# facebook/zstd

Hardware: NVIDIA H100
Metric: compress GB/s (input) at level 1 (higher is better)
Workload: dtype u8

## Files before the change

zstd_b200/csrc/zb_device.cuh:

```cuda
#ifndef ZB_DEVICE_CUH
#define ZB_DEVICE_CUH
#include <cuda_runtime.h>
#include "zb_common.h"

#define ZB_FULL 0xFFFFFFFFu

__device__ __forceinline__ u32 zb_ld32u(const u8* p)
{
    const u32* q = (const u32*)((uintptr_t)p & ~(uintptr_t)3);
    u32 const sh = ((u32)(uintptr_t)p & 3u) * 8u;
    u32 const a = __ldg(q);
    u32 const b = __ldg(sh ? q + 1 : q);
    return __funnelshift_r(a, b, sh);
}
__device__ __forceinline__ u64 zb_ld64u(const u8* p)
{
    const u32* q = (const u32*)((uintptr_t)p & ~(uintptr_t)3);
    u32 const sh = ((u32)(uintptr_t)p & 3u) * 8u;
    u32 const a = __ldg(q);
    u32 const b = __ldg(q + 1);
    u32 const c = __ldg(sh ? q + 2 : q + 1);
    u32 const lo = __funnelshift_r(a, b, sh);
    u32 const hi = __funnelshift_r(b, c, sh);
    return ((u64)hi << 32) | lo;
}

__device__ __forceinline__ u32 zb_ld32w2(const u8* p)
{
    const u32* q = (const u32*)((uintptr_t)p & ~(uintptr_t)3);
    u32 const sh = ((u32)(uintptr_t)p & 3u) * 8u;
    return __funnelshift_r(__ldg(q), __ldg(q + 1), sh);
}
__device__ __forceinline__ u64 zb_ld64w3(const u8* p)
{
    const u32* q = (const u32*)((uintptr_t)p & ~(uintptr_t)3);
    u32 const sh = ((u32)(uintptr_t)p & 3u) * 8u;
    u32 const a = __ldg(q), b = __ldg(q + 1), c = __ldg(q + 2);
    return ((u64)__funnelshift_r(b, c, sh) << 32) | __funnelshift_r(a, b, sh);
}
struct ZbSeg { const u8* lo; const u8* hi; u32 split; };

template <bool DICT> __device__ __forceinline__ const u8* zb_seg_ptr(const ZbSeg& s, u32 rel)
{
    if (DICT) return (rel < s.split ? s.lo : s.hi) + rel;
    return s.hi + rel;
}
template <bool DICT> __device__ __forceinline__ u8 zb_seg_byte(const ZbSeg& s, u32 rel) { return *zb_seg_ptr<DICT>(s, rel); }

template <bool DICT> __device__ __forceinline__ u64 zb_seg_ld64(const ZbSeg& s, u32 rel)
{
    if (DICT && rel < s.split && rel + 12u > s.split) {
        u64 v = 0;
#pragma unroll
        for (u32 i = 0; i < 8u; i++) v |= (u64)zb_seg_byte<true>(s, rel + i) << (8u * i);
        return v;
    }
    return zb_ld64w3(zb_seg_ptr<DICT>(s, rel));
}
template <bool DICT> __device__ __forceinline__ u64 zb_seg_ld64x(const ZbSeg& s, u32 rel)
{
    if (DICT && rel < s.split && rel + 12u > s.split) {
        u64 v = 0;
#pragma unroll
        for (u32 i = 0; i < 8u; i++) v |= (u64)zb_seg_byte<true>(s, rel + i) << (8u * i);
        return v;
    }
    return zb_ld64u(zb_seg_ptr<DICT>(s, rel));
}
template <bool DICT> __device__ __forceinline__ u32 zb_seg_ld32(const ZbSeg& s, u32 rel) { return (u32)zb_seg_ld64<DICT>(s, rel); }
template <bool DICT> __device__ __forceinline__ void zb_seg_pre_cur(const ZbSeg& sg, u32 x, u32* pre, u32* cur)
{
    u32 const s = x >= 4u ? 0u : 4u - x;
    u64 const w = zb_seg_ld64<DICT>(sg, x + s - 4u);
    *pre = (u32)(w << (8u * s));
    *cur = (u32)(w >> (32u - 8u * s));
}

__device__ __forceinline__ u32 zb_hash(u64 v, u32 mls, u32 hBits)
{
    switch (mls) {
    default:
    case 4: return ((u32)v * 2654435761u) >> (32 - hBits);
    case 5: return (u32)(((v << 24) * 889523592379ull) >> (64 - hBits));
    case 6: return (u32)(((v << 16) * 227718039650203ull) >> (64 - hBits));
    case 7: return (u32)(((v << 8) * 58295818150454627ull) >> (64 - hBits));
    case 8: return (u32)((v * 0xCF1BBCDCB7A56463ull) >> (64 - hBits));
    }
}

__device__ __forceinline__ u32 zb_hb32(u32 v) { return 31u - (u32)__clz((int)v); }

__device__ __forceinline__ u64 zbx_rotl(u64 x, int r) { return (x << r) | (x >> (64 - r)); }
#define ZBX_P1 0x9E3779B185EBCA87ull
#define ZBX_P2 0xC2B2AE3D27D4EB4Full
#define ZBX_P3 0x165667B19E3779F9ull
#define ZBX_P4 0x85EBCA77C2B2AE63ull
#define ZBX_P5 0x27D4EB2F165667C5ull
__device__ __forceinline__ u64 zbx_round(u64 acc, u64 in) { return zbx_rotl(acc + in * ZBX_P2, 31) * ZBX_P1; }
__device__ __forceinline__ u64 zbx_merge(u64 h, u64 v) { return (h ^ zbx_round(0, v)) * ZBX_P1 + ZBX_P4; }

#endif
```

zstd_b200/csrc/zb_match.cu:

```cuda
#include "zb_device.cuh"
#include "zb_kernels.h"
#include "zb_merge.cuh"

#ifndef WALK_FAST_BC
#define WALK_FAST_BC 1
#endif

template <bool DICT>
__device__ __forceinline__ u32 zb_count_fwd(const ZbSeg& sg, u32 a, u32 offset, u32 be, u32 lane)
{
    u32 fwd = 0;
    while (true) {
        u32 const pa = a + fwd + 8u * lane;
        u32 m;
        if (pa + 8u <= be) {
            u64 const x = zb_seg_ld64x<DICT>(sg, pa) ^ zb_seg_ld64x<DICT>(sg, pa - offset);
            m = x ? (u32)((__ffsll((long long)x) - 1) >> 3) : 8u;
        } else {
            m = 0;
            while (pa + m < be && zb_seg_byte<DICT>(sg, pa + m) == zb_seg_byte<DICT>(sg, pa + m - offset)) m++;
        }
        u32 const inc = __ballot_sync(ZB_FULL, m != 8u);
        if (inc == 0) { fwd += 256u; continue; }
        int const f = __ffs((int)inc) - 1;
        fwd += 8u * (u32)f + __shfl_sync(ZB_FULL, m, f);
        return fwd;
    }
}

template <bool DICT>
__device__ __forceinline__ u32 zb_back_coop(const ZbSeg& sg, u32 probe, u32 offset, u32 anchor, u32 lane)
{
    u32 back = 0;
    while (true) {
        u32 const k = back + lane + 1u;
        bool const ok = (probe >= anchor + k) && (probe >= offset + k)
                     && (zb_seg_byte<DICT>(sg, probe - k) == zb_seg_byte<DICT>(sg, probe - offset - k));
        u32 const okb = __ballot_sync(ZB_FULL, ok);
        u32 const cnt = (okb == ZB_FULL) ? 32u : (u32)(__ffs((int)~okb) - 1);
        back += cnt;
        if (cnt < 32u) return back;
    }
}

__device__ __forceinline__ u64 zb_pack_raw(u32 off, u32 mlen, u32 msRel) { return (u64)off | ((u64)mlen << 24) | ((u64)msRel << 42); }
#define ZB_RAW_OFF(r)  ((u32)(r) & 0xFFFFFFu)
#define ZB_RAW_MLEN(r) ((u32)((r) >> 24) & 0x3FFFFu)
#define ZB_RAW_MS(r)   ((u32)((r) >> 42))

#define ZB_TAG_MASK ((1u << ZB_TAG_BITS) - 1u)
__device__ __forceinline__ u32 zb_walk_key(u32 x) { return (x | (ZB_BATCH - 1u)) - (x & (ZB_BATCH - 1u)); }
__device__ __forceinline__ u32 zb_walk_entry(u32 h, u32 x) { return ((zb_walk_key(x) + 1u) << ZB_TAG_BITS) | (h & ZB_TAG_MASK); }
__device__ __forceinline__ u32 zb_walk_cand(u32 c, u32 h, u32 x)
{
    u32 const px = zb_walk_key((c >> ZB_TAG_BITS) - 1u);
    return (((c ^ h) & ZB_TAG_MASK) == 0u && px < x) ? x - px : 0u;
}

template <int P>
__device__ __forceinline__ u32 zb_walk_pattern_res(u32 r0, u32 step)
{
    if (step <= 2u) return (1u << P) - 1u;
    u32 m = 3u >> (r0 < 2u ? r0 : 2u);
    u32 nxt = step - r0;
#pragma unroll
    for (int k = 0; k < (P + 2) / 3; k++) {
        m |= 3u << (nxt < 31u ? nxt : 31u);
        nxt += step;
    }
    return m & ((1u << P) - 1u);
}
__device__ __forceinline__ u32 zb_walk_residue(u32 rel0, u32 step)
{
    u32 const q = (u32)__fdividef((float)rel0, (float)step);
    int r = (int)rel0 - (int)(q * step);
    if (r < 0) r += (int)step; else if (r >= (int)step) r -= (int)step;
    return (u32)r;
}

#define ZB_WALK_NWR(P) ((P) == 1 ? 2 : ((P) + 7 + 3) / 4)
template <int MLS, int P, bool INTERIOR>
__device__ __forceinline__ bool zb_walk_batch(u32* __restrict__ table, u32 xa, const u32 (&wrd)[ZB_WALK_NWR(P)], u32 pat,
                                              u32 N, u32 shift, u32 D, u32 total, u32 xLow, u32 xEnd,
                                              const u8* fbase, const u8* dbase, bool output, u16* __restrict__ distRow, u32* __restrict__ farRow)
{
    u32 h[P], bkt[P], dOld[P];
    bool act[P];
    {   u32 const rel0 = xa - shift;
        bool const slow = !INTERIOR && ((xa < xLow) || (D != 0u && rel0 < D && rel0 + P + 7u > D) || (rel0 + P + 7u > total));
        u32 old[P];
#pragma unroll
        for (int i = 0; i < P; i++) {
            u32 const x = xa + (u32)i, rel = x - shift;
            act[i] = INTERIOR ? true : ((x >= xLow) && (rel + 8u <= total) && !(rel < D && rel + 8u > D));
            u64 v;
            if (slow) v = act[i] ? zb_ld64u((rel < D ? dbase : fbase) + rel) : 0ull;
            else {
                constexpr int NWR = ZB_WALK_NWR(P);
                int const wi = i >> 2; u32 const sh = 8u * (u32)(i & 3);
                int const w2 = wi + 2 < NWR ? wi + 2 : NWR - 1;
                u32 const lo = (i & 3) ? __funnelshift_r(wrd[wi], wrd[wi + 1], sh) : wrd[wi];
                u32 const hi = (i & 3) ? __funnelshift_r(wrd[wi + 1], wrd[w2], sh) : wrd[wi + 1];
                v = ((u64)hi << 32) | lo;
            }
            h[i] = zb_hash(v, MLS, 32u);
            bkt[i] = __umulhi(h[i], N);
            old[i] = act[i] ? table[bkt[i]] : 0u;
        }
#pragma unroll
        for (int i = 0; i < P; i++) dOld[i] = zb_walk_cand(old[i], h[i], xa + (u32)i);
    }
    u32 anyOld = 0;
#pragma unroll
    for (int i = 0; i < P; i++) anyOld |= dOld[i];
    bool const anyHit = __syncthreads_or(anyOld != 0u) != 0;
#if WALK_FAST_BC
    u32 const Y1 = zb_walk_key(xa) + 1u;
#pragma unroll
    for (int i = 0; i < P; i++)
        if (act[i] && dOld[i] == 0u && ((pat >> i) & 1u)) atomicMax(&table[bkt[i]], ((Y1 - (u32)i) << ZB_TAG_BITS) | (h[i] & ZB_TAG_MASK));
    __syncthreads();
    u32 d[P];
#pragma unroll
    for (int i = 0; i < P; i++) {
        d[i] = dOld[i];
        if (act[i] && d[i] == 0u) {
            u32 const c = table[bkt[i]];
            int const dd = (int)((c >> ZB_TAG_BITS) - Y1 + (u32)i);
            d[i] = ((((c ^ h[i]) & ZB_TAG_MASK) == 0u) && dd > 0) ? (u32)dd : 0u;
        }
    }
#else
#pragma unroll
    for (int i = 0; i < P; i++)
        if (act[i] && dOld[i] == 0u && ((pat >> i) & 1u)) atomicMax(&table[bkt[i]], zb_walk_entry(h[i], xa + (u32)i));
    __syncthreads();
    u32 d[P];
#pragma unroll
    for (int i = 0; i < P; i++) {
        d[i] = dOld[i];
        if (act[i] && d[i] == 0u) d[i] = zb_walk_cand(table[bkt[i]], h[i], xa + (u32)i);
    }
#endif
    if (output && (INTERIOR || xa < xEnd)) {
        u32 anyFar = 0;
#pragma unroll
        for (int i = 0; i < P; i++) anyFar |= d[i] >= ZB_FAR ? 1u : 0u;
        if (anyFar) {
#pragma unroll
            for (int i = 0; i < P; i++) if (d[i] >= ZB_FAR) { if (INTERIOR || xa + (u32)i < xEnd) farRow[i] = d[i]; d[i] = ZB_FAR; }
        }
        bool vec = false;
        if constexpr (P == 16) { if (INTERIOR || xa + 16u <= xEnd) { uint4* const o4 = reinterpret_cast<uint4*>(distRow);
                                     o4[0] = make_uint4(d[0] | (d[1] << 16), d[2] | (d[3] << 16), d[4] | (d[5] << 16), d[6] | (d[7] << 16));
                                     o4[1] = make_uint4(d[8] | (d[9] << 16), d[10] | (d[11] << 16), d[12] | (d[13] << 16), d[14] | (d[15] << 16)); vec = true; } }
        if constexpr (P == 8) { if (INTERIOR || xa + 8u <= xEnd) { *reinterpret_cast<uint4*>(distRow) = make_uint4(d[0] | (d[1] << 16), d[2] | (d[3] << 16), d[4] | (d[5] << 16), d[6] | (d[7] << 16)); vec = true; } }
        if constexpr (P == 4) { if (INTERIOR || xa + 4u <= xEnd) { *reinterpret_cast<uint2*>(distRow) = make_uint2(d[0] | (d[1] << 16), d[2] | (d[3] << 16)); vec = true; } }
        if constexpr (P == 2) { if (INTERIOR || xa + 2u <= xEnd) { *reinterpret_cast<u32*>(distRow) = d[0] | (d[1] << 16); vec = true; } }
        if (!vec) {
#pragma unroll
            for (int i = 0; i < P; i++) if (xa + (u32)i < xEnd) distRow[i] = (u16)d[i];
        }
    }
    return anyHit;
}

#ifndef WALK_STEADY
#define WALK_STEADY 1
#endif
#ifndef WALK_P_SMALL
#define WALK_P_SMALL 8
#endif
#ifndef WALK_P_MID
#define WALK_P_MID 4
#endif
#ifndef WALK_MINB_SMALL
#define WALK_MINB_SMALL 4
#endif
template <int MLS, int P>
__global__ void __launch_bounds__(ZB_BATCH / P, P == WALK_P_SMALL ? WALK_MINB_SMALL : 1)
zb_walk_kernel(const u8* __restrict__ src, const u8* __restrict__ dictEnd, const ZbChunk* __restrict__ chunks, u32 insStep, u32 N, ZbStrides sd,
               u32 slotFirstBlock, u16* __restrict__ dist, u32* __restrict__ far,
               const u32* __restrict__ imageIn, u32* __restrict__ imageOut)
{
    constexpr u32 THREADS = ZB_BATCH / P;
    extern __shared__ __align__(16) u32 table[];
    u32 const t = threadIdx.x;
    ZbChunk const cd = chunks[blockIdx.x];
    bool const buildImage = imageOut != nullptr;
    u32 const D = cd.dictLen;
    u32 const H = cd.histLen;
    u32 const total = buildImage ? D : H + cd.size;
    bool const fromImage = imageIn != nullptr && D != 0u && !buildImage;
    u32 const shift = (ZB_BATCH - (D % ZB_BATCH)) % ZB_BATCH;
    const u8* const fbase = src + cd.srcOff - H;
    const u8* const dbase = dictEnd - D;

    if (fromImage) for (u32 i = t; i < N; i += THREADS) table[i] = __ldg(imageIn + i);
    else           for (u32 i = t; i < N; i += THREADS) table[i] = 0u;
    __syncthreads();

    u32 const xEnd = total + shift;
    u32 const xLow = (fromImage ? D : 0u) + shift;
    u32 x0 = xLow & ~(ZB_BATCH - 1u);
    u32 const xIntLo = ((D + shift) > xLow ? (D + shift) : xLow);
    u32 const xIntLoB = (xIntLo + ZB_BATCH - 1u) & ~(ZB_BATCH - 1u);
    constexpr u32 NW = (P + 7u + 3u + 3u) / 4u;
    constexpr int NWR = ZB_WALK_NWR(P);
    u32 const xIntHi = xEnd >= (ZB_BATCH + 4u * NW) ? (xEnd + P - 4u * NW) & ~(ZB_BATCH - 1u) : 0u;

    auto fetch = [&](u32 xb, u32 (&a)[NW], u32& sh) {
        u32 const xa = xb + P * t;
#pragma unroll
        for (u32 k = 0; k < NW; k++) a[k] = 0u;
        sh = 0u;
        if (xb >= xIntLoB && xb + ZB_BATCH <= xIntHi) {
            const u8* const ad = fbase + (xa - shift);
            const u32* const p = reinterpret_cast<const u32*>((uintptr_t)ad & ~(uintptr_t)3);
            sh = ((u32)(uintptr_t)ad & 3u) * 8u;
#pragma unroll
            for (u32 k = 0; k < NW; k++) a[k] = __ldg(p + k);
            return;
        }
        if (xa + P <= xLow || xa >= xEnd) return;
        u32 const rel = xa - shift;
        bool const slow = (xa < xLow) || (D != 0u && rel < D && rel + P + 7u > D) || (rel + P + 7u > total);
        if (slow) return;
        const u8* const ad = (rel < D ? dbase : fbase) + rel;
        const u32* const p = reinterpret_cast<const u32*>((uintptr_t)ad & ~(uintptr_t)3);
        u32 const al = (u32)(uintptr_t)ad & 3u;
        sh = al * 8u;
#pragma unroll
        for (u32 k = 0; k < NW; k++) a[k] = (al + P + 7u > 4u * k) ? __ldg(p + k) : 0u;
    };
    u32 rawA[NW], rawB[NW], shA, shB;
    fetch(x0, rawA, shA);
    fetch(x0 + ZB_BATCH, rawB, shB);
    u32 const blockMask = (1u << cd.blockLog) - 1u;
    u32 const stepInc = ZB_BATCH % insStep;
    u32 r0 = (x0 + P * t + insStep * ZB_BATCH - shift) % insStep;
    u32 li = shift;
    auto doBatch = [&](u32 (&raw)[NW], u32& sh) {
        u32 const xa = x0 + P * t;
        u32 cur[NWR];
#pragma unroll
        for (int k = 0; k < NWR; k++) cur[k] = __funnelshift_r(raw[k], (u32)k + 1u < NW ? raw[(u32)k + 1u < NW ? k + 1 : k] : 0u, sh);
        fetch(x0 + 2u * ZB_BATCH, raw, sh);
        if (D != 0u && x0 >= D + shift && li < D + shift) li = D + shift;
        u32 const sWalk = x0 > xLow ? x0 : xLow;
        u32 const step = insStep + ((sWalk - li) >> 7);
        u32 const pat = zb_walk_pattern_res<P>(step == insStep ? r0 : zb_walk_residue(xa - shift, step), step);
        bool const output = !buildImage && x0 >= H + shift;
        u32 const qb0 = x0 - shift - H;
        size_t const idx = output ? (size_t)(cd.firstBlock - slotFirstBlock + (qb0 >> cd.blockLog)) * sd.dist + (qb0 & blockMask) + P * t : 0;
        bool hit;
        if (x0 >= xIntLoB && x0 + ZB_BATCH <= xIntHi)
            hit = zb_walk_batch<MLS, P, true>(table, xa, cur, pat, N, shift, D, total, xLow, xEnd, fbase, dbase, output, dist + idx, far + idx);
        else
            hit = zb_walk_batch<MLS, P, false>(table, xa, cur, pat, N, shift, D, total, xLow, xEnd, fbase, dbase, output, dist + idx, far + idx);
        if (hit) li = x0 + ZB_BATCH;
        r0 += stepInc; if (r0 >= insStep) r0 -= insStep;
        x0 += ZB_BATCH;
    };
    const u8* const tbase = fbase + P * t - shift;
    u16* const distT = dist + P * t;
    u32* const farT = far + P * t;
    auto steadyBatch = [&](u32 (&raw)[NW], u32 const sh) {
        u32 const xa = x0 + P * t;
        u32 cur[NWR];
#pragma unroll
        for (int k = 0; k < NWR; k++) cur[k] = __funnelshift_r(raw[k], (u32)k + 1u < NW ? raw[(u32)k + 1u < NW ? k + 1 : k] : 0u, sh);
        {   const u32* const pw = reinterpret_cast<const u32*>((uintptr_t)(tbase + x0 + 2u * ZB_BATCH) & ~(uintptr_t)3);
#pragma unroll
            for (u32 k = 0; k < NW; k++) raw[k] = __ldg(pw + k);
        }
        u32 const step = insStep + ((x0 - li) >> 7);
        u32 const pat = zb_walk_pattern_res<P>(step == insStep ? r0 : zb_walk_residue(xa - shift, step), step);
        bool const output = !buildImage && x0 >= H + shift;
        u32 const qb0 = x0 - shift - H;
        size_t const row = output ? (size_t)(cd.firstBlock - slotFirstBlock + (qb0 >> cd.blockLog)) * sd.dist + (qb0 & blockMask) : 0;
        if (zb_walk_batch<MLS, P, true>(table, xa, cur, pat, N, shift, D, total, xLow, xEnd, fbase, dbase, output, distT + row, farT + row)) li = x0 + ZB_BATCH;
        r0 += stepInc; if (r0 >= insStep) r0 -= insStep;
        x0 += ZB_BATCH;
    };
    while (x0 < xEnd) {
        if (WALK_STEADY && x0 >= xIntLoB && x0 + 4u * ZB_BATCH <= xIntHi) {
            if (D != 0u && li < D + shift) li = D + shift;
            do { steadyBatch(rawA, shA); steadyBatch(rawB, shB); } while (x0 + 4u * ZB_BATCH <= xIntHi);
        }
        doBatch(rawA, shA);
        if (x0 >= xEnd) break;
        doBatch(rawB, shB);
    }
    if (buildImage) { __syncthreads(); for (u32 i = t; i < N; i += THREADS) imageOut[i] = table[i]; }
}

#ifndef PARSE_WARPS
#define PARSE_WARPS 8
#endif
#ifndef PARSE_MIN_CTAS
#define PARSE_MIN_CTAS 6
#endif
__device__ __forceinline__ u32 zb_dist_at(const u16* __restrict__ d16, const u32* __restrict__ far, u32 i)
{
    u32 const d = d16[i];
    return d == ZB_FAR ? far[i] : d;
}

template <bool DICT>
__global__ void __launch_bounds__(32 * PARSE_WARPS, DICT ? (40 / PARSE_WARPS) : PARSE_MIN_CTAS)
zb_parse_kernel(const u8* __restrict__ src, const u8* __restrict__ dictEnd, const ZbBlock* __restrict__ blocks, u32 nbBlocks, ZbParams prm, ZbStrides sd,
                const u16* __restrict__ dist, const u32* __restrict__ far, u64* __restrict__ seqs, ZbBlockMeta* __restrict__ meta, ZbSegMeta* __restrict__ segmeta)
{
    u32 const lane = threadIdx.x & 31u;
    u32 const g = blockIdx.x * PARSE_WARPS + (threadIdx.x >> 5);
    u32 const segs = (sd.dist + ZB_PARSE_SEG - 1u) / ZB_PARSE_SEG;
    u32 const b = g / segs, k = g % segs;
    if (b >= nbBlocks) return;
    ZbBlock const bd = blocks[b];
    u64* const myseq = seqs + (size_t)b * sd.seq + (size_t)k * (ZB_PARSE_SEG / 4u);
    const u16* const mydist = dist + (size_t)b * sd.dist;
    const u32* const myfar = far + (size_t)b * sd.dist;
    const u8* const base = src + bd.srcOff - bd.histLen;
    u32 const bs = bd.histLen, blockEnd = bd.histLen + bd.size;
    ZbSeg sg; sg.hi = base; sg.lo = base; sg.split = 0;
    if (DICT && (bd.flags & ZB_FLAG_DICT)) { sg.lo = dictEnd - bd.dictLen; sg.split = bd.dictLen; }

    if (bd.size < 7u) {
        if (lane == 0 && k == 0) {
            ZbBlockMeta m; m.nbSeq = 0; m.litSize = bd.size; m.litSecSize = 0; m.bodySize = bd.size;
            m.type = ZB_BT_RAW; m.forceRaw = 1; m.rleByte = 0; m.pad = 0;
            meta[b] = m;
        }
        return;
    }
    u32 const ss = bs + k * ZB_PARSE_SEG;
    if (ss >= blockEnd) {
        if (lane == 0) { ZbSegMeta z; z.nbSeq = 0; z.pad[0] = z.pad[1] = z.pad[2] = 0; segmeta[(size_t)b * segs + k] = z; }
        return;
    }
    u32 const se = min(ss + ZB_PARSE_SEG, blockEnd);
    u32 const be = blockEnd;

    u32 ip = ss, anchor = ss, searchStart = ss;
    u32 rep1 = 0, rep2 = 0, nbSeq = 0;
    if ((bd.flags & ZB_FLAG_FIRST) && k == 0u) { rep1 = prm.startRep[0]; rep2 = prm.startRep[1]; }

    while (ip < se && ip + 8u <= be) {
        u32 const step = prm.stepSize + ((ip - searchStart) >> 7);
        u32 const p = ip + (lane >> 1) * step + (lane & 1u);
        bool const act = (p < se) && (p + 8u <= be);
        u32 const pp = act ? p : ip;
        u32 const d16 = act ? (u32)mydist[pp - bs] : 0u;
        bool const v3 = (lane == 0u) && (ip == anchor) && (rep2 != 0u);
        bool const v2 = act && rep1 != 0u && p >= rep1;
        u32 pre, cur;
        zb_seg_pre_cur<DICT>(sg, pp, &pre, &cur);
        u32 const cur2 = DICT ? zb_seg_ld32<DICT>(sg, v2 ? pp - rep1 : pp) : zb_ld32w2(sg.hi + (v2 ? pp - rep1 : pp));
        u32 cur3 = ~cur;
        if (ip == anchor && rep2 != 0u) cur3 = (u32)zb_seg_ld64x<DICT>(sg, v3 ? pp - rep2 : pp);
        u32 const d = d16 == ZB_FAR ? myfar[pp - bs] : d16;
        bool const v1 = act && d != 0u && p >= d;
        u32 const hit = (v3 && cur3 == cur) ? 3u : ((v2 && cur2 == cur) ? 2u : (v1 ? 1u : 0u));
        u32 myback = 0, mymore = 0;
        if (hit == 2u) {
            u32 pre2, unused;
            zb_seg_pre_cur<DICT>(sg, p - rep1, &pre2, &unused);
            u32 const x = pre ^ pre2;
            u32 const bm = x ? ((u32)__clz((int)x) >> 3) : 4u;
            u32 lim = p - anchor; lim = lim < 4u ? lim : 4u;
            u32 const src0 = p - rep1; lim = lim < src0 ? lim : src0;
            myback = bm < lim ? bm : lim;
            mymore = (bm == 4u && lim == 4u) ? 1u : 0u;
        }
        u32 tent = __ballot_sync(ZB_FULL, hit != 0u);
        u32 probe = 0, wtype = 0, offset = 0, back = 0, fwdFrom4 = 0;
        bool found = false;
        while (tent) {
            int const winner = __ffs((int)tent) - 1;
            probe = __shfl_sync(ZB_FULL, p, winner);
            wtype = __shfl_sync(ZB_FULL, hit, winner);
            u32 const wd = __shfl_sync(ZB_FULL, d, winner);
            back = __shfl_sync(ZB_FULL, myback, winner);
            u32 more = __shfl_sync(ZB_FULL, mymore, winner);
            offset = (wtype == 3u) ? rep2 : ((wtype == 2u) ? rep1 : wd);
            if (wtype == 1u) {
                u32 const f0 = zb_count_fwd<DICT>(sg, probe, offset, be, lane);
                if (f0 < 4u) { tent &= ~(1u << winner); continue; }
                fwdFrom4 = f0 - 4u;
                more = 1u;
            } else {
                fwdFrom4 = zb_count_fwd<DICT>(sg, probe + 4u, offset, be, lane);
            }
            if (more) back += zb_back_coop<DICT>(sg, probe - back, offset, anchor, lane);
            found = true;
            break;
        }
        if (!found) { ip += 16u * step; continue; }
        u32 const ms = probe - back;
        u32 const mlen = back + 4u + fwdFrom4;
        if (wtype == 3u) { u32 const t = rep2; rep2 = rep1; rep1 = t; }
        else if (wtype == 1u) { rep2 = rep1; rep1 = offset; }
        if (lane == 0) myseq[nbSeq] = zb_pack_raw(offset, mlen, ms - bs);
        nbSeq++;
        ip = ms + mlen; anchor = ip; searchStart = ip;
    }
    if (lane == 0) { ZbSegMeta z; z.nbSeq = nbSeq; z.pad[0] = z.pad[1] = z.pad[2] = 0; segmeta[(size_t)b * segs + k] = z; }
}

template <bool DICT>
__global__ void __launch_bounds__(32 * PARSE_WARPS)
zb_parse_dfast_kernel(const u8* __restrict__ src, const u8* __restrict__ dictEnd, const ZbBlock* __restrict__ blocks, u32 nbBlocks, ZbParams prm, ZbStrides sd,
                      const u16* __restrict__ distLong, const u32* __restrict__ farLong, const u16* __restrict__ distShort, const u32* __restrict__ farShort,
                      u64* __restrict__ seqs, ZbBlockMeta* __restrict__ meta, ZbSegMeta* __restrict__ segmeta)
{
    u32 const lane = threadIdx.x & 31u;
    u32 const g = blockIdx.x * PARSE_WARPS + (threadIdx.x >> 5);
    u32 const segs = (sd.dist + ZB_PARSE_SEG - 1u) / ZB_PARSE_SEG;
    u32 const b = g / segs, k = g % segs;
    if (b >= nbBlocks) return;
    ZbBlock const bd = blocks[b];
    u64* const myseq = seqs + (size_t)b * sd.seq + (size_t)k * (ZB_PARSE_SEG / 4u);
    const u16* const dLp = distLong + (size_t)b * sd.dist;
    const u32* const fLp = farLong + (size_t)b * sd.dist;
    const u16* const dSp = distShort + (size_t)b * sd.dist;
    const u32* const fSp = farShort + (size_t)b * sd.dist;
    const u8* const base = src + bd.srcOff - bd.histLen;
    u32 const bs = bd.histLen, blockEnd = bd.histLen + bd.size;
    ZbSeg sg; sg.hi = base; sg.lo = base; sg.split = 0;
    if (DICT && (bd.flags & ZB_FLAG_DICT)) { sg.lo = dictEnd - bd.dictLen; sg.split = bd.dictLen; }

    if (bd.size < 7u) {
        if (lane == 0 && k == 0) {
            ZbBlockMeta m; m.nbSeq = 0; m.litSize = bd.size; m.litSecSize = 0; m.bodySize = bd.size;
            m.type = ZB_BT_RAW; m.forceRaw = 1; m.rleByte = 0; m.pad = 0;
            meta[b] = m;
        }
        return;
    }
    u32 const ss = bs + k * ZB_PARSE_SEG;
    if (ss >= blockEnd) {
        if (lane == 0) { ZbSegMeta z; z.nbSeq = 0; z.pad[0] = z.pad[1] = z.pad[2] = 0; segmeta[(size_t)b * segs + k] = z; }
        return;
    }
    u32 const se = min(ss + ZB_PARSE_SEG, blockEnd);
    u32 const be = blockEnd;
    u32 ip = ss, anchor = ss, searchStart = ss;
    u32 rep1 = 0, rep2 = 0, nbSeq = 0;
    if ((bd.flags & ZB_FLAG_FIRST) && k == 0u) { rep1 = prm.startRep[0]; rep2 = prm.startRep[1]; }

    while (ip < se && ip + 9u <= be) {
        u32 const step = 1u + ((ip - searchStart) >> 8);
        u32 const p = ip + lane * step;
        bool const act = (p < se) && (p + 9u <= be);
        u32 const pp = act ? p : ip;
        u32 dL = act ? zb_dist_at(dLp, fLp, pp - bs) : 0u;
        u32 dS = act ? zb_dist_at(dSp, fSp, pp - bs) : 0u;
        u32 dL1 = act ? zb_dist_at(dLp, fLp, pp + 1u - bs) : 0u;
        if (dL > pp) dL = 0u;
        if (dS > pp) dS = 0u;
        if (dL1 > pp + 1u) dL1 = 0u;
        u64 const w = zb_seg_ld64x<DICT>(sg, pp);
        u32 const cur = (u32)w, cur1 = (u32)(w >> 8);
        bool const v2 = act && rep1 != 0u && (p + 1u >= rep1);
        u32 const r2 = (u32)zb_seg_ld64x<DICT>(sg, v2 ? pp + 1u - rep1 : pp);
        u32 r3 = ~cur;
        bool const v3 = (lane == 0u) && (ip == anchor) && (rep2 != 0u);
        if (ip == anchor && rep2 != 0u) r3 = (u32)zb_seg_ld64x<DICT>(sg, v3 ? pp - rep2 : pp);
        u32 hit = (v3 && r3 == cur) ? 3u : ((v2 && r2 == cur1) ? 2u : (dL ? 1u : (dS ? 4u : 0u)));
        u32 tent = __ballot_sync(ZB_FULL, hit != 0u);
        u32 ms = 0, offset = 0, mlen = 0, wtype = 0;
        bool found = false;
        while (tent) {
            int const winner = __ffs((int)tent) - 1;
            u32 const probe = __shfl_sync(ZB_FULL, p, winner);
            wtype = __shfl_sync(ZB_FULL, hit, winner);
            u32 const wL = __shfl_sync(ZB_FULL, dL, winner), wS = __shfl_sync(ZB_FULL, dS, winner), wL1 = __shfl_sync(ZB_FULL, dL1, winner);
            if (wtype == 3u) { ms = probe; offset = rep2; mlen = 4u + zb_count_fwd<DICT>(sg, probe + 4u, rep2, be, lane); found = true; break; }
            if (wtype == 2u) { ms = probe + 1u; offset = rep1; mlen = 4u + zb_count_fwd<DICT>(sg, probe + 5u, rep1, be, lane); found = true; break; }
            if (wtype == 1u) {
                u32 const f0 = zb_count_fwd<DICT>(sg, probe, wL, be, lane);
                if (f0 >= 8u) {
                    u32 const back = zb_back_coop<DICT>(sg, probe, wL, anchor, lane);
                    ms = probe - back; offset = wL; mlen = back + f0; found = true; break;
                }
                if (lane == (u32)winner) hit = dS ? 4u : 0u;
                if (wS == 0u) { tent &= ~(1u << winner); }
                continue;
            }
            {   u32 const f0 = zb_count_fwd<DICT>(sg, probe, wS, be, lane);
                if (f0 < 4u) { tent &= ~(1u << winner); if (lane == (u32)winner) hit = 0u; continue; }
                u32 mp = probe, mo = wS, ml = f0;
                if (wL1) {
                    u32 const f1 = zb_count_fwd<DICT>(sg, probe + 1u, wL1, be, lane);
                    if (f1 >= 8u && f1 > ml) { mp = probe + 1u; mo = wL1; ml = f1; }
                }
                u32 const back = zb_back_coop<DICT>(sg, mp, mo, anchor, lane);
                ms = mp - back; offset = mo; mlen = back + ml; wtype = 1u; found = true; break;
            }
        }
        if (!found) { ip += 32u * step; continue; }
        if (wtype == 3u) { u32 const t = rep2; rep2 = rep1; rep1 = t; }
        else if (wtype == 1u) { rep2 = rep1; rep1 = offset; }
        if (lane == 0) myseq[nbSeq] = zb_pack_raw(offset, mlen, ms - bs);
        nbSeq++;
        ip = ms + mlen; anchor = ip; searchStart = ip;
    }
    if (lane == 0) { ZbSegMeta z; z.nbSeq = nbSeq; z.pad[0] = z.pad[1] = z.pad[2] = 0; segmeta[(size_t)b * segs + k] = z; }
}

struct ZbRepHist { u32 r1, r2, r3; };
__device__ __forceinline__ u32 zb_rep_code(ZbRepHist& h, u32 off, u32 ll)
{
    u32 code;
    if (ll > 0u) {
        if (off == h.r1) return 1u;
        if (off == h.r2) { code = 2u; h.r2 = h.r1; h.r1 = off; return code; }
        if (off == h.r3) { code = 3u; h.r3 = h.r2; h.r2 = h.r1; h.r1 = off; return code; }
    } else {
        if (off == h.r2) { code = 1u; h.r2 = h.r1; h.r1 = off; return code; }
        if (off == h.r3) { code = 2u; h.r3 = h.r2; h.r2 = h.r1; h.r1 = off; return code; }
        if (h.r1 > 1u && off == h.r1 - 1u) { code = 3u; h.r3 = h.r2; h.r2 = h.r1; h.r1 = off; return code; }
    }
    h.r3 = h.r2; h.r2 = h.r1; h.r1 = off;
    return off + 3u;
}

#ifndef MERGE_MIN_CTAS
#define MERGE_MIN_CTAS 6
#endif
#define SEG_SLOTS (ZB_PARSE_SEG / 4u)

__device__ __forceinline__ u32 zb_block_excl(bool flag, u32* wsum, u32* total)
{
    u32 const lane = threadIdx.x & 31u, warp = threadIdx.x >> 5;
    u32 const bal = __ballot_sync(ZB_FULL, flag);
    if (lane == 0u) wsum[warp] = __popc(bal);
    __syncthreads();
    u32 before = __popc(bal & ((1u << lane) - 1u)), t = 0;
    for (u32 w = 0; w < MERGE_THREADS / 32u; w++) { if (w < warp) before += wsum[w]; t += wsum[w]; }
    __syncthreads();
    *total = t;
    return before;
}

__device__ __forceinline__ void zb_ldm_clip(u32 ms, u32 me, const u64* L, u32 nL, u32* ms2, u32* me2, u32* next, bool* kept)
{
    u32 lo = 0, hi = nL;
    while (lo < hi) { u32 const mid = (lo + hi) >> 1; if (ZB_LDM_START(L[mid]) <= ms) lo = mid + 1u; else hi = mid; }
    bool clipped = false;
    if (lo > 0u && ZB_LDM_START(L[lo - 1u]) + ZB_LDM_LEN(L[lo - 1u]) > ms) { ms = ZB_LDM_START(L[lo - 1u]) + ZB_LDM_LEN(L[lo - 1u]); clipped = true; }
    if (lo < nL && ZB_LDM_START(L[lo]) < me) { me = ZB_LDM_START(L[lo]); clipped = true; }
    *ms2 = ms; *me2 = me; *next = lo;
    *kept = me > ms && (!clipped || me - ms >= 4u);
}
__device__ u32 zb_ldm_overlay(const u64* __restrict__ P, u32 nP, const u64* __restrict__ L, u32 nL, u32* __restrict__ kp, u64* __restrict__ out,
                              u32* wsum, u32* sEnd, u32& carry)
{
    u32 const tid = threadIdx.x;
    u32 base = 0;
    for (u32 i0 = 0; i0 < nP; i0 += MERGE_THREADS) {
        u32 const i = i0 + tid;
        u32 ms2, me2, nx; bool kept = false;
        if (i < nP) { u64 const r = P[i]; zb_ldm_clip(ZB_RAW_MS(r), ZB_RAW_MS(r) + ZB_RAW_MLEN(r), L, nL, &ms2, &me2, &nx, &kept); }
        u32 t;
        u32 const before = zb_block_excl(kept, wsum, &t);
        if (i < nP) kp[i] = base + before;
        base += t;
    }
    if (tid == 0) kp[nP] = base;
    __syncthreads();
    for (u32 i = tid; i < nP; i += MERGE_THREADS) {
        u64 const r = P[i];
        u32 ms2, me2, nx; bool kept;
        zb_ldm_clip(ZB_RAW_MS(r), ZB_RAW_MS(r) + ZB_RAW_MLEN(r), L, nL, &ms2, &me2, &nx, &kept);
        if (kept) out[kp[i] + nx] = zb_pack_ldm(ms2, me2 - ms2, ZB_RAW_OFF(r));
    }
    for (u32 k = tid; k < nL; k += MERGE_THREADS) {
        u32 const s = ZB_LDM_START(L[k]);
        u32 lo = 0, hi = nP;
        while (lo < hi) { u32 const mid = (lo + hi) >> 1; if (ZB_RAW_MS(P[mid]) < s) lo = mid + 1u; else hi = mid; }
        out[k + kp[lo]] = L[k];
    }
    u32 const n = base + nL;
    __syncthreads();
    if (tid == 0) carry = 0;
    for (u32 o0 = 0; o0 < n; o0 += MERGE_THREADS) {
        u32 const o = o0 + tid;
        u64 const m = o < n ? out[o] : 0ull;
        sEnd[tid] = ZB_LDM_START(m) + ZB_LDM_LEN(m);
        __syncthreads();
        u32 const prevEnd = tid ? sEnd[tid - 1u] : carry;
        if (o < n) out[o] = zb_pack_seq(ZB_LDM_OFF(m), ZB_LDM_START(m) - prevEnd, ZB_LDM_LEN(m));
        __syncthreads();
        if (tid == MERGE_THREADS - 1u) carry = sEnd[tid];
        __syncthreads();
    }
    return n;
}

template <bool LDM>
__global__ void __launch_bounds__(MERGE_THREADS, MERGE_MIN_CTAS)
zb_merge_segments_kernel(const u8* __restrict__ src, const ZbBlock* __restrict__ blocks, ZbParams prm, ZbStrides sd, const ZbSegMeta* __restrict__ segmeta,
                         u64* __restrict__ seqs, u8* __restrict__ lits, ZbBlockMeta* __restrict__ meta,
                         ZbLdmView ldm, u32* __restrict__ farScratch, u16* __restrict__ distScratch)
{
    __shared__ u32 sPos[MERGE_TILE], sLit[MERGE_TILE], sLen[MERGE_TILE], sOff[MERGE_TILE];
    __shared__ u32 wsumL[MERGE_THREADS / 32], wsumA[MERGE_THREADS / 32], wmaxU[MERGE_THREADS / 32], wmaxK[MERGE_THREADS / 32];
    __shared__ u32 sR2[MERGE_TILE], sRep[3];
    __shared__ u32 baseL, baseA, carryEnd;
    __shared__ u32 gFirst[ZB_PARSE_SEGS], gCnt[ZB_PARSE_SEGS], gBase[ZB_PARSE_SEGS], gCur[ZB_PARSE_SEGS], gPm[ZB_PARSE_SEGS], gPl[ZB_PARSE_SEGS];
    __shared__ u32 gTotal;
    u32 const b = blockIdx.x, tid = threadIdx.x, lane = tid & 31u, warp = tid >> 5;
    ZbBlock const bd = blocks[b];
    if (bd.size < 7u) return;
    u64* const myseq = seqs + (size_t)b * sd.seq;
    u8*  const mylit = lits + (size_t)b * sd.lit;
    const u8* const in = src + bd.srcOff;
    u32 const segs = (bd.size + ZB_PARSE_SEG - 1u) / ZB_PARSE_SEG;
    u32 const segStride = (sd.dist + ZB_PARSE_SEG - 1u) / ZB_PARSE_SEG;
    if (warp == 0u) {
        u32 nb = 0; u64 r0 = 0, rl = 0;
        if (lane < segs) {
            nb = segmeta[(size_t)b * segStride + lane].nbSeq;
            if (nb) { r0 = myseq[(size_t)lane * SEG_SLOTS]; rl = myseq[(size_t)lane * SEG_SLOTS + nb - 1u]; }
        }
        u32 cur = 0, total = 0;
        for (u32 k = 0; k < segs; k++) {
            u32 const n = __shfl_sync(ZB_FULL, nb, (int)k);
            u64 r = __shfl_sync(ZB_FULL, r0, (int)k);
            u64 const last = __shfl_sync(ZB_FULL, rl, (int)k);
            u32 f = 0, pm = 0, pl = 0;
            while (f < n) {
                u32 const ms = ZB_RAW_MS(r), ml = ZB_RAW_MLEN(r);
                if (ms + ml <= cur || (ms < cur && ms + ml - cur < 3u)) { f++; if (f < n) r = myseq[(size_t)k * SEG_SLOTS + f]; continue; }
                if (ms < cur) { pm = cur; pl = ms + ml - cur; } else { pm = ms; pl = ml; }
                break;
            }
            if (lane == 0u) { gFirst[k] = f; gCnt[k] = n - f; gBase[k] = total; gCur[k] = cur; gPm[k] = pm; gPl[k] = pl; }
            if (f < n) { cur = (f == n - 1u) ? pm + pl : ZB_RAW_MS(last) + ZB_RAW_MLEN(last); total += n - f; }
        }
        if (lane == 0u) gTotal = total;
    }
    __syncthreads();
    u32 nbSeq;
    if constexpr (LDM) {
        u64* const P = reinterpret_cast<u64*>(farScratch + (size_t)b * sd.dist);
#pragma unroll 1
        for (u32 k = 0; k < segs; k++) {
            u32 const f = gFirst[k], cnt = gCnt[k];
            const u64* const sfrom = myseq + (size_t)k * SEG_SLOTS + f;
            for (u32 i = tid; i < cnt; i += MERGE_THREADS) {
                u64 r = sfrom[i];
                if (i == 0u) r = zb_pack_raw(ZB_RAW_OFF(r), gPl[k], gPm[k]);
                P[gBase[k] + i] = r;
            }
        }
        __syncthreads();
        nbSeq = zb_ldm_overlay(P, gTotal, ldm.match + ldm.first[b], ldm.cnt[b], reinterpret_cast<u32*>(distScratch + (size_t)b * sd.dist), myseq,
                               wsumA, sPos, carryEnd);
        __syncthreads();
    } else {
#pragma unroll 1
    for (u32 k = 0; k < segs; k++) {
        u32 const f = gFirst[k], cnt = gCnt[k];
        const u64* const sfrom = myseq + (size_t)k * SEG_SLOTS + f;
        u64* const sto = myseq + gBase[k];
        for (u32 c0 = 0; c0 < cnt; c0 += MERGE_THREADS) {
            u32 const i = c0 + tid;
            u64 r = 0; u32 ms = 0, ml = 0;
            if (i < cnt) { r = sfrom[i]; ms = ZB_RAW_MS(r); ml = ZB_RAW_MLEN(r); if (i == 0u) { ms = gPm[k]; ml = gPl[k]; } }
            u32 const myEnd = ms + ml;
            u32 prevEnd = __shfl_up_sync(ZB_FULL, myEnd, 1);
            if (lane == 31u) wsumL[warp] = myEnd;
            __syncthreads();
            if (lane == 0u) prevEnd = warp ? wsumL[warp - 1u] : (c0 ? carryEnd : gCur[k]);
            __syncthreads();
            if (i < cnt) sto[i] = zb_pack_seq(ZB_RAW_OFF(r), ms - prevEnd, ml);
            if (tid == MERGE_THREADS - 1u) carryEnd = myEnd;
            __syncthreads();
        }
    }
    nbSeq = gTotal;
    }
    zb_merge_codes(prm.codeRep[0], prm.codeRep[1], prm.codeRep[2], (bd.flags & ZB_FLAG_FIRST) != 0u, myseq, mylit, in, nbSeq, bd.size, meta + b,
                   sPos, sLit, sLen, sOff, sR2, sRep, wsumL, wsumA, wmaxU, wmaxK, baseL, baseA);
}

__global__ void __launch_bounds__(MERGE_THREADS)
zb_merge_small_kernel(const u8* __restrict__ src, const ZbBlock* __restrict__ blocks, u32 nbBlocks, ZbParams prm, ZbStrides sd, const ZbSegMeta* __restrict__ segmeta,
                      u64* __restrict__ seqs, u8* __restrict__ lits, ZbBlockMeta* __restrict__ meta)
{
    u32 const lane = threadIdx.x & 31u;
    u32 const b = blockIdx.x * (MERGE_THREADS / 32u) + (threadIdx.x >> 5);
    if (b >= nbBlocks) return;
    ZbBlock const bd = blocks[b];
    if (bd.size < 7u) return;
    u64* const myseq = seqs + (size_t)b * sd.seq;
    u8* const mylit = lits + (size_t)b * sd.lit;
    const u8* const in = src + bd.srcOff;
    u32 const nbSeq = segmeta[b].nbSeq;
    ZbRepHist hist; hist.r1 = 0; hist.r2 = 0; hist.r3 = 0;
    if (bd.flags & ZB_FLAG_FIRST) { hist.r1 = prm.codeRep[0]; hist.r2 = prm.codeRep[1]; hist.r3 = prm.codeRep[2]; }
    u32 posL = 0, posA = 0;
    for (u32 t0 = 0; t0 < nbSeq; t0 += 32u) {
        u32 const i = t0 + lane;
        u64 const r = (i < nbSeq) ? myseq[i] : 0ull;
        u32 const ms = ZB_RAW_MS(r), ml = ZB_RAW_MLEN(r), off = ZB_RAW_OFF(r);
        u32 const myEnd = (i < nbSeq) ? ms + ml : 0u;
        u32 prevEnd = __shfl_up_sync(ZB_FULL, myEnd, 1);
        if (lane == 0u) prevEnd = posA;
        u32 const ll = (i < nbSeq) ? ms - prevEnd : 0u;
        u32 const adv = ll + ((i < nbSeq) ? ml : 0u);
        u32 inL = ll;
#pragma unroll
        for (u32 o = 1; o < 32u; o <<= 1) { u32 const x = __shfl_up_sync(ZB_FULL, inL, o); if (lane >= o) inL += x; }
        u32 code = 0;
        u32 const cnt = min(32u, nbSeq - t0);
        for (u32 j = 0; j < cnt; j++) {
            u32 const o = __shfl_sync(ZB_FULL, off, (int)j), l = __shfl_sync(ZB_FULL, ll, (int)j);
            u32 const c = zb_rep_code(hist, o, l);
            if (lane == j) code = c;
        }
        if (i < nbSeq) {
            const u8* const from = in + prevEnd;
            u8* const to = mylit + posL + inL - ll;
            for (u32 x = 0; x < ll; x++) to[x] = from[x];
            myseq[i] = zb_pack_seq(code, ll, ml);
        }
        posL += __shfl_sync(ZB_FULL, inL, 31);
        posA = __shfl_sync(ZB_FULL, myEnd, (int)(cnt - 1u));
        (void)adv;
    }
    u32 const lastLits = bd.size - posA;
    for (u32 x = lane; x < lastLits; x += 32u) mylit[posL + x] = in[posA + x];
    if (lane == 0) {
        ZbBlockMeta m; m.nbSeq = nbSeq; m.litSize = posL + lastLits; m.litSecSize = 0; m.bodySize = 0;
        m.type = ZB_BT_COMPRESSED; m.forceRaw = 0; m.rleByte = 0; m.pad = 0;
        meta[b] = m;
    }
}

template <int MLS, int P>
static cudaError_t zb_launch_walk_p(const u8* d_src, const u8* d_dictEnd, const ZbChunk* d_chunks, u32 nbChunks, u32 N, u32 insStep, const ZbStrides& sd,
                                    u32 slotFirstBlock, u16* d_dist, u32* d_far, const u32* d_imageIn, u32* d_imageOut, cudaStream_t stream)
{
    cudaError_t const e = cudaFuncSetAttribute(zb_walk_kernel<MLS, P>, cudaFuncAttributeMaxDynamicSharedMemorySize, 226 * 1024);
    if (e != cudaSuccess) return e;
    zb_walk_kernel<MLS, P><<<nbChunks, ZB_BATCH / P, (size_t)N * 4u, stream>>>(d_src, d_dictEnd, d_chunks, insStep, N, sd, slotFirstBlock, d_dist, d_far, d_imageIn, d_imageOut);
    return cudaGetLastError();
}
template <int MLS>
static cudaError_t zb_launch_walk_m(const u8* d_src, const u8* d_dictEnd, const ZbChunk* d_chunks, u32 nbChunks, u32 N, u32 insStep, const ZbStrides& sd,
                                    u32 slotFirstBlock, u16* d_dist, u32* d_far, const u32* d_imageIn, u32* d_imageOut, cudaStream_t stream)
{
    size_t const smem = (size_t)N * 4u;
    if (smem <= 56u * 1024u)  return zb_launch_walk_p<MLS, WALK_P_SMALL>(d_src, d_dictEnd, d_chunks, nbChunks, N, insStep, sd, slotFirstBlock, d_dist, d_far, d_imageIn, d_imageOut, stream);
    if (smem <= 113u * 1024u) return zb_launch_walk_p<MLS, WALK_P_MID>(d_src, d_dictEnd, d_chunks, nbChunks, N, insStep, sd, slotFirstBlock, d_dist, d_far, d_imageIn, d_imageOut, stream);
    return zb_launch_walk_p<MLS, 1>(d_src, d_dictEnd, d_chunks, nbChunks, N, insStep, sd, slotFirstBlock, d_dist, d_far, d_imageIn, d_imageOut, stream);
}
static cudaError_t zb_launch_walk(const u8* d_src, const u8* d_dictEnd, const ZbChunk* d_chunks, u32 nbChunks, u32 mls, u32 N, u32 insStep, const ZbStrides& sd,
                                  u32 slotFirstBlock, u16* d_dist, u32* d_far, const u32* d_imageIn, u32* d_imageOut, cudaStream_t stream)
{
    switch (mls) {
    case 4: return zb_launch_walk_m<4>(d_src, d_dictEnd, d_chunks, nbChunks, N, insStep, sd, slotFirstBlock, d_dist, d_far, d_imageIn, d_imageOut, stream);
    case 5: return zb_launch_walk_m<5>(d_src, d_dictEnd, d_chunks, nbChunks, N, insStep, sd, slotFirstBlock, d_dist, d_far, d_imageIn, d_imageOut, stream);
    case 6: return zb_launch_walk_m<6>(d_src, d_dictEnd, d_chunks, nbChunks, N, insStep, sd, slotFirstBlock, d_dist, d_far, d_imageIn, d_imageOut, stream);
    case 7: return zb_launch_walk_m<7>(d_src, d_dictEnd, d_chunks, nbChunks, N, insStep, sd, slotFirstBlock, d_dist, d_far, d_imageIn, d_imageOut, stream);
    default: return zb_launch_walk_m<8>(d_src, d_dictEnd, d_chunks, nbChunks, N, insStep, sd, slotFirstBlock, d_dist, d_far, d_imageIn, d_imageOut, stream);
    }
}

extern "C" cudaError_t zb_launch_dict_image(const u8* d_dictEnd, const ZbChunk* d_dictChunk, const ZbParams* prm, u32* d_image, cudaStream_t stream)
{
    ZbStrides sd; sd.dist = ZB_BLOCK_MAX; sd.seq = ZB_SEQ_STRIDE; sd.lit = ZB_LIT_STRIDE; sd.body = ZB_BODY_STRIDE; sd.state = ZB_STATE_STRIDE;
    cudaError_t e = zb_launch_walk(nullptr, d_dictEnd, d_dictChunk, 1, prm->mls, prm->tableN, prm->insStep, sd, 0, nullptr, nullptr, nullptr, d_image, stream);
    if (e == cudaSuccess && prm->strategy == 2)
        e = zb_launch_walk(nullptr, d_dictEnd, d_dictChunk, 1, 8, prm->tableNLong, prm->insStep, sd, 0, nullptr, nullptr, nullptr, d_image + prm->tableN, stream);
    return e;
}

extern "C" cudaError_t zb_launch_match(const u8* d_src, const u8* d_dictEnd, const u32* d_image, const ZbBlock* d_blocks, u32 nbBlocks,
                                       const ZbChunk* d_chunks, u32 nbChunks, u32 slotFirstBlock, const ZbParams* prm, const ZbStrides* sdp,
                                       u16* d_dist, u32* d_far, u16* d_dist2, u32* d_far2, u64* d_seqs, u8* d_lits, ZbBlockMeta* d_meta, ZbSegMeta* d_segmeta,
                                       cudaEvent_t evMid, cudaStream_t stream, const ZbLdmView* ldm)
{
    if (nbBlocks == 0) return cudaSuccess;
    ZbStrides const sd = *sdp;
    cudaError_t e;
    u32 const segs = (sd.dist + ZB_PARSE_SEG - 1u) / ZB_PARSE_SEG;
    u32 const sgrid = (u32)(((u64)nbBlocks * segs + PARSE_WARPS - 1) / PARSE_WARPS);
    if (prm->strategy == 2) {
        e = zb_launch_walk(d_src, d_dictEnd, d_chunks, nbChunks, 8, prm->tableNLong, prm->insStep, sd, slotFirstBlock, d_dist, d_far, d_image ? d_image + prm->tableN : nullptr, nullptr, stream); if (e != cudaSuccess) return e;
        e = zb_launch_walk(d_src, d_dictEnd, d_chunks, nbChunks, prm->mls, prm->tableN, prm->insStep, sd, slotFirstBlock, d_dist2, d_far2, d_image, nullptr, stream); if (e != cudaSuccess) return e;
        if (evMid) cudaEventRecord(evMid, stream);
        if (d_dictEnd) zb_parse_dfast_kernel<true><<<sgrid, 32 * PARSE_WARPS, 0, stream>>>(d_src, d_dictEnd, d_blocks, nbBlocks, *prm, sd, d_dist, d_far, d_dist2, d_far2, d_seqs, d_meta, d_segmeta);
        else           zb_parse_dfast_kernel<false><<<sgrid, 32 * PARSE_WARPS, 0, stream>>>(d_src, nullptr, d_blocks, nbBlocks, *prm, sd, d_dist, d_far, d_dist2, d_far2, d_seqs, d_meta, d_segmeta);
    } else {
        e = zb_launch_walk(d_src, d_dictEnd, d_chunks, nbChunks, prm->mls, prm->tableN, prm->insStep, sd, slotFirstBlock, d_dist, d_far, d_image, nullptr, stream); if (e != cudaSuccess) return e;
        if (evMid) cudaEventRecord(evMid, stream);
        if (d_dictEnd) zb_parse_kernel<true><<<sgrid, 32 * PARSE_WARPS, 0, stream>>>(d_src, d_dictEnd, d_blocks, nbBlocks, *prm, sd, d_dist, d_far, d_seqs, d_meta, d_segmeta);
        else           zb_parse_kernel<false><<<sgrid, 32 * PARSE_WARPS, 0, stream>>>(d_src, nullptr, d_blocks, nbBlocks, *prm, sd, d_dist, d_far, d_seqs, d_meta, d_segmeta);
    }
    if (segs == 1u && sd.dist <= 8192u)
        zb_merge_small_kernel<<<(nbBlocks + MERGE_THREADS / 32u - 1u) / (MERGE_THREADS / 32u), MERGE_THREADS, 0, stream>>>(d_src, d_blocks, nbBlocks, *prm, sd, d_segmeta, d_seqs, d_lits, d_meta);
    else if (ldm)
        zb_merge_segments_kernel<true><<<nbBlocks, MERGE_THREADS, 0, stream>>>(d_src, d_blocks, *prm, sd, d_segmeta, d_seqs, d_lits, d_meta, *ldm, d_far, d_dist);
    else
        zb_merge_segments_kernel<false><<<nbBlocks, MERGE_THREADS, 0, stream>>>(d_src, d_blocks, *prm, sd, d_segmeta, d_seqs, d_lits, d_meta, ZbLdmView(), nullptr, nullptr);
    return cudaGetLastError();
}
```

Measured before the change: 93.03.

## Streamline walk batch hashing, candidate decoding and distance output

Replaces the 64-bit multiply hash with a templated 32-bit formulation built from mulhi and low multiplies. The batch-reversed key becomes a simple XOR. After the atomicMax, the candidate distance is recovered with a single subtract and funnel shift instead of tag compare and signed arithmetic. Atomics are issued unconditionally with a zero value when inactive, non-output batches return early, and the far check becomes a warp vote. The goal is fewer instructions and less branching in the hot hash-table walk, at the cost of more atomic traffic from the dummy atomics and subtle correctness risks in the new candidate decoding.

```diff
diff --git a/zstd_b200/csrc/zb_device.cuh b/zstd_b200/csrc/zb_device.cuh
--- a/zstd_b200/csrc/zb_device.cuh
+++ b/zstd_b200/csrc/zb_device.cuh
@@ -76,16 +76,23 @@
     *cur = (u32)(w >> (32u - 8u * s));
 }
 
-__device__ __forceinline__ u32 zb_hash(u64 v, u32 mls, u32 hBits)
+__host__ __device__ __forceinline__ u32 zb_mulhi(u32 a, u32 b)
 {
-    switch (mls) {
-    default:
-    case 4: return ((u32)v * 2654435761u) >> (32 - hBits);
-    case 5: return (u32)(((v << 24) * 889523592379ull) >> (64 - hBits));
-    case 6: return (u32)(((v << 16) * 227718039650203ull) >> (64 - hBits));
-    case 7: return (u32)(((v << 8) * 58295818150454627ull) >> (64 - hBits));
-    case 8: return (u32)((v * 0xCF1BBCDCB7A56463ull) >> (64 - hBits));
-    }
+#ifdef __CUDA_ARCH__
+    return __umulhi(a, b);
+#else
+    return (u32)(((u64)a * b) >> 32);
+#endif
+}
+
+template <int MLS>
+__host__ __device__ __forceinline__ u32 zb_hash32(u32 lo, u32 hi)
+{
+    static_assert(MLS >= 4 && MLS <= 8, "minimum match length 4..8");
+    if (MLS == 4) return lo * 2654435761u;
+    constexpr u64 C = MLS == 5 ? 889523592379ull << 24 : MLS == 6 ? 227718039650203ull << 16
+                    : MLS == 7 ? 58295818150454627ull << 8 : 0xCF1BBCDCB7A56463ull;
+    return zb_mulhi(lo, (u32)C) + lo * (u32)(C >> 32) + hi * (u32)C;
 }
 
 __device__ __forceinline__ u32 zb_hb32(u32 v) { return 31u - (u32)__clz((int)v); }
diff --git a/zstd_b200/csrc/zb_match.cu b/zstd_b200/csrc/zb_match.cu
--- a/zstd_b200/csrc/zb_match.cu
+++ b/zstd_b200/csrc/zb_match.cu
@@ -1,10 +1,6 @@
 #include "zb_device.cuh"
 #include "zb_kernels.h"
 #include "zb_merge.cuh"
-
-#ifndef WALK_FAST_BC
-#define WALK_FAST_BC 1
-#endif
 
 template <bool DICT>
 __device__ __forceinline__ u32 zb_count_fwd(const ZbSeg& sg, u32 a, u32 offset, u32 be, u32 lane)
@@ -49,12 +45,11 @@
 #define ZB_RAW_MS(r)   ((u32)((r) >> 42))
 
 #define ZB_TAG_MASK ((1u << ZB_TAG_BITS) - 1u)
-__device__ __forceinline__ u32 zb_walk_key(u32 x) { return (x | (ZB_BATCH - 1u)) - (x & (ZB_BATCH - 1u)); }
-__device__ __forceinline__ u32 zb_walk_entry(u32 h, u32 x) { return ((zb_walk_key(x) + 1u) << ZB_TAG_BITS) | (h & ZB_TAG_MASK); }
-__device__ __forceinline__ u32 zb_walk_cand(u32 c, u32 h, u32 x)
+__device__ __forceinline__ u32 zb_walk_key(u32 x) { return x ^ (ZB_BATCH - 1u); }
+__device__ __forceinline__ u32 zb_walk_cand_prior(u32 c, u32 h, u32 x)
 {
     u32 const px = zb_walk_key((c >> ZB_TAG_BITS) - 1u);
-    return (((c ^ h) & ZB_TAG_MASK) == 0u && px < x) ? x - px : 0u;
+    return (((c ^ h) & ZB_TAG_MASK) == 0u && c != 0u) ? x - px : 0u;
 }
 
 template <int P>
@@ -88,79 +83,61 @@
     bool act[P];
     {   u32 const rel0 = xa - shift;
         bool const slow = !INTERIOR && ((xa < xLow) || (D != 0u && rel0 < D && rel0 + P + 7u > D) || (rel0 + P + 7u > total));
-        u32 old[P];
 #pragma unroll
         for (int i = 0; i < P; i++) {
             u32 const x = xa + (u32)i, rel = x - shift;
             act[i] = INTERIOR ? true : ((x >= xLow) && (rel + 8u <= total) && !(rel < D && rel + 8u > D));
-            u64 v;
-            if (slow) v = act[i] ? zb_ld64u((rel < D ? dbase : fbase) + rel) : 0ull;
+            u32 lo, hi;
+            if (slow) { u64 const v = act[i] ? zb_ld64u((rel < D ? dbase : fbase) + rel) : 0ull; lo = (u32)v; hi = (u32)(v >> 32); }
             else {
                 constexpr int NWR = ZB_WALK_NWR(P);
                 int const wi = i >> 2; u32 const sh = 8u * (u32)(i & 3);
                 int const w2 = wi + 2 < NWR ? wi + 2 : NWR - 1;
-                u32 const lo = (i & 3) ? __funnelshift_r(wrd[wi], wrd[wi + 1], sh) : wrd[wi];
-                u32 const hi = (i & 3) ? __funnelshift_r(wrd[wi + 1], wrd[w2], sh) : wrd[wi + 1];
-                v = ((u64)hi << 32) | lo;
+                lo = (i & 3) ? __funnelshift_r(wrd[wi], wrd[wi + 1], sh) : wrd[wi];
+                hi = (i & 3) ? __funnelshift_r(wrd[wi + 1], wrd[w2], sh) : wrd[wi + 1];
             }
-            h[i] = zb_hash(v, MLS, 32u);
+            h[i] = zb_hash32<MLS>(lo, hi);
             bkt[i] = __umulhi(h[i], N);
-            old[i] = act[i] ? table[bkt[i]] : 0u;
-        }
-#pragma unroll
-        for (int i = 0; i < P; i++) dOld[i] = zb_walk_cand(old[i], h[i], xa + (u32)i);
+            dOld[i] = zb_walk_cand_prior(act[i] ? table[bkt[i]] : 0u, h[i], x);
+        }
     }
     u32 anyOld = 0;
 #pragma unroll
     for (int i = 0; i < P; i++) anyOld |= dOld[i];
     bool const anyHit = __syncthreads_or(anyOld != 0u) != 0;
-#if WALK_FAST_BC
-    u32 const Y1 = zb_walk_key(xa) + 1u;
-#pragma unroll
-    for (int i = 0; i < P; i++)
-        if (act[i] && dOld[i] == 0u && ((pat >> i) & 1u)) atomicMax(&table[bkt[i]], ((Y1 - (u32)i) << ZB_TAG_BITS) | (h[i] & ZB_TAG_MASK));
+    u32 const Y1s = (zb_walk_key(xa) + 1u) << ZB_TAG_BITS;
+    u32 e[P];
+#pragma unroll
+    for (int i = 0; i < P; i++) {
+        e[i] = (Y1s - ((u32)i << ZB_TAG_BITS)) | (h[i] & ZB_TAG_MASK);
+        atomicMax(&table[bkt[i]], (act[i] && dOld[i] == 0u && ((pat >> i) & 1u)) ? e[i] : 0u);
+    }
     __syncthreads();
-    u32 d[P];
+    if (!output) return anyHit;
+    u32 d[P], orD = 0;
 #pragma unroll
     for (int i = 0; i < P; i++) {
-        d[i] = dOld[i];
-        if (act[i] && d[i] == 0u) {
-            u32 const c = table[bkt[i]];
-            int const dd = (int)((c >> ZB_TAG_BITS) - Y1 + (u32)i);
-            d[i] = ((((c ^ h[i]) & ZB_TAG_MASK) == 0u) && dd > 0) ? (u32)dd : 0u;
-        }
-    }
-#else
-#pragma unroll
-    for (int i = 0; i < P; i++)
-        if (act[i] && dOld[i] == 0u && ((pat >> i) & 1u)) atomicMax(&table[bkt[i]], zb_walk_entry(h[i], xa + (u32)i));
-    __syncthreads();
-    u32 d[P];
-#pragma unroll
-    for (int i = 0; i < P; i++) {
-        d[i] = dOld[i];
-        if (act[i] && d[i] == 0u) d[i] = zb_walk_cand(table[bkt[i]], h[i], xa + (u32)i);
-    }
-#endif
-    if (output && (INTERIOR || xa < xEnd)) {
-        u32 anyFar = 0;
-#pragma unroll
-        for (int i = 0; i < P; i++) anyFar |= d[i] >= ZB_FAR ? 1u : 0u;
-        if (anyFar) {
-#pragma unroll
-            for (int i = 0; i < P; i++) if (d[i] >= ZB_FAR) { if (INTERIOR || xa + (u32)i < xEnd) farRow[i] = d[i]; d[i] = ZB_FAR; }
-        }
-        bool vec = false;
-        if constexpr (P == 16) { if (INTERIOR || xa + 16u <= xEnd) { uint4* const o4 = reinterpret_cast<uint4*>(distRow);
-                                     o4[0] = make_uint4(d[0] | (d[1] << 16), d[2] | (d[3] << 16), d[4] | (d[5] << 16), d[6] | (d[7] << 16));
-                                     o4[1] = make_uint4(d[8] | (d[9] << 16), d[10] | (d[11] << 16), d[12] | (d[13] << 16), d[14] | (d[15] << 16)); vec = true; } }
-        if constexpr (P == 8) { if (INTERIOR || xa + 8u <= xEnd) { *reinterpret_cast<uint4*>(distRow) = make_uint4(d[0] | (d[1] << 16), d[2] | (d[3] << 16), d[4] | (d[5] << 16), d[6] | (d[7] << 16)); vec = true; } }
-        if constexpr (P == 4) { if (INTERIOR || xa + 4u <= xEnd) { *reinterpret_cast<uint2*>(distRow) = make_uint2(d[0] | (d[1] << 16), d[2] | (d[3] << 16)); vec = true; } }
-        if constexpr (P == 2) { if (INTERIOR || xa + 2u <= xEnd) { *reinterpret_cast<u32*>(distRow) = d[0] | (d[1] << 16); vec = true; } }
-        if (!vec) {
-#pragma unroll
-            for (int i = 0; i < P; i++) if (xa + (u32)i < xEnd) distRow[i] = (u16)d[i];
-        }
+        u32 const c = table[bkt[i]] - e[i];
+        u32 const r = __funnelshift_r(c, c, ZB_TAG_BITS);
+        d[i] = (act[i] && r < ZB_BATCH) ? r : dOld[i];
+        orD |= d[i];
+    }
+    bool const mine = INTERIOR || xa < xEnd;
+    if (__any_sync(ZB_FULL, mine && orD >= ZB_FAR)) {
+#pragma unroll
+        for (int i = 0; i < P; i++) if (d[i] >= ZB_FAR) { if (mine && (INTERIOR || xa + (u32)i < xEnd)) farRow[i] = d[i]; d[i] = ZB_FAR; }
+    }
+    if (!mine) return anyHit;
+    auto pk = [&](int i) { return __byte_perm(d[i], d[i + 1], 0x5410); };
+    bool vec = false;
+    if constexpr (P == 16) { if (INTERIOR || xa + 16u <= xEnd) { uint4* const o4 = reinterpret_cast<uint4*>(distRow);
+                                 o4[0] = make_uint4(pk(0), pk(2), pk(4), pk(6)); o4[1] = make_uint4(pk(8), pk(10), pk(12), pk(14)); vec = true; } }
+    if constexpr (P == 8) { if (INTERIOR || xa + 8u <= xEnd) { *reinterpret_cast<uint4*>(distRow) = make_uint4(pk(0), pk(2), pk(4), pk(6)); vec = true; } }
+    if constexpr (P == 4) { if (INTERIOR || xa + 4u <= xEnd) { *reinterpret_cast<uint2*>(distRow) = make_uint2(pk(0), pk(2)); vec = true; } }
+    if constexpr (P == 2) { if (INTERIOR || xa + 2u <= xEnd) { *reinterpret_cast<u32*>(distRow) = pk(0); vec = true; } }
+    if (!vec) {
+#pragma unroll
+        for (int i = 0; i < P; i++) if (xa + (u32)i < xEnd) distRow[i] = (u16)d[i];
     }
     return anyHit;
 }
```

Result: faster. 95.89, median of 6 (+3.1%).
